# BoloniniD/CSWin-UNet

Hardware: AMD Instinct MI355X
Metric: training images/sec (224x224, cswin_tiny) (higher is better)
Workload: dtype f32; 1 GPU; cswin_tiny_224_lite, synthetic 224x224 9-class, bs=24/GPU, fp32 matmul, fwd + 0.4CE+0.6Dice + bwd + SGD(momentum) step, drop_path 0.2; global_batch=24, img_size=224, parallelism=dp1, hip_graph=True

## Files before the change

### cswin_unet_amd/_lib.py

```python
import ctypes
import os
from ctypes import c_char_p, c_double, c_float, c_int, c_long, c_size_t, c_void_p

import torch

_HERE = os.path.dirname(os.path.abspath(__file__))
LIB_PATH = os.path.join(_HERE, "libcswin_hip.so")

P, I, F, SZ, L, D = c_void_p, c_int, c_float, c_size_t, c_long, c_double

ABI_VERSION = 4

SIGNATURES = {
    "cswin_last_error": (c_char_p, []),
    "cswin_abi_version": (I, []),
    "cswin_device_ok": (I, []),
    "cswin_attn_fwd": (I, [P, P, P, P, P, P, I, I, I, I, P, P, I, F, F, ctypes.c_ulonglong, P, I, P]),
    "cswin_attn_bwd_workspace": (SZ, [I, I, I, I, P, P, I]),
    "cswin_attn_bwd": (I, [P, P, P, P, P, P, P, P, P, P, SZ, I, I, I, I, P, P, I, F, P, F, ctypes.c_ulonglong, P, I, P]),
    "cswin_img2windows": (I, [P, P, I, I, I, I, I, I, P]),
    "cswin_windows2img": (I, [P, P, I, I, I, I, I, I, P]),
    "cswin_layernorm_fwd": (I, [P, P, P, P, P, P, I, I, F, I, P]),
    "cswin_layernorm_bwd_workspace": (SZ, [I, I]),
    "cswin_layernorm_bwd": (I, [P, P, P, P, P, P, P, P, P, P, SZ, I, I, P, P, P]),
    "cswin_linear_fwd": (I, [P, P, I, P, P, P, P, P, P, I, I, I, I, I, I, P]),
    "cswin_linear_bwd_data": (I, [P, P, P, P, I, P, P, I, P, I, I, I, I, I, P]),
    "cswin_linear_bwd_weight_workspace": (SZ, [I, I, I]),
    "cswin_linear_bwd_weight": (I, [P, P, P, I, P, I, P, P, P, SZ, I, I, I, P, I, P]),
    "cswin_linear_bwd_weight_batch": (I, [P, I, P, P, I, P]),
    "cswin_linear_bwd_tail": (I, [P, P, P, I, I, I, P, I, P, P, I, P]),
    "cswin_linear_bwd_weight_batch_masked": (I, [P, I, P, P, I, P, P, P]),
    "cswin_linear_bwd_tail_masked": (I, [P, P, P, I, I, I, P, I, P, P, I, P, P, P]),
    "cswin_rows_sum_multi": (I, [P, I, P]),
    "cswin_conv_tok_fwd": (I, [P, P, P, P, I, I, I, I, I, I, I, I, I, P]),
    "cswin_conv_tok_bwd_data": (I, [P, P, P, I, I, I, I, I, I, I, I, I, P]),
    "cswin_conv_tok_bwd_weight_workspace": (SZ, [I, I, I, I, I, I, I, I]),
    "cswin_conv_tok_bwd_weight": (I, [P, P, P, P, P, SZ, I, I, I, I, I, I, I, I, I, P, I, P]),
    "cswin_conv_weight_permute": (I, [P, P, P, I, I, I, I, P]),
    "cswin_conv_weight_unpermute": (I, [P, P, I, I, I, I, P]),
    "cswin_conv_weight_flipT": (I, [P, P, I, I, I, P]),
# ... 195 lines not shown
```

### cswin_unet_amd/csrc/gemm.hip

```cpp
#include <stdlib.h>

#include <type_traits>
#include "common.h"
#include "gemm_epilogue.h"

int cswin_gemm16(int mode, int epi_mode, const void* A, const void* B, const void* epilogue, int M, int NO, int R, void* stream);
int cswin_wgrad16_batch(const cswin_wgrad_desc* d, int n, const int* splits, const int* rows_per_split, const cswin_reduce_job* pending,
                        int npending, void* stream, long long* stamps);

namespace {

constexpr int BKMAX = 64;

typedef __bf16 bf16x8 __attribute__((ext_vector_type(8)));

#define CSWIN_CHECK_PRECISION(p, who) CSWIN_REQUIRE((p) == 0 || (p) == 1, CSWIN_ERR_UNSUPPORTED, who ": precision %d (0 = fp32, 1 = bf16 operands)", (p))

struct PlainSrc {
    const float* p; long ld; int rows, cols;
    const float* row_scale; int rows_per_sample;
    int bf16;
    static constexpr bool fast_div = false;
    struct Row { const float* base; float s; };
    typedef int Col;
// ... 10 lines not shown
template <class S> __device__ __forceinline__ bool src_is_bf16(const S&) { return false; }
__device__ __forceinline__ bool src_is_bf16(const PlainSrc& s) { return s.bf16 != 0; }
template <class S> __device__ __forceinline__ u32x2 src_load4_bf16(const S&, const float*) { return u32x2{0u, 0u}; }
__device__ __forceinline__ u32x2 src_load4_bf16(const PlainSrc& s, const float* p) {
    return *reinterpret_cast<const u32x2*>(reinterpret_cast<const __bf16*>(s.p) + (p - s.p));
}
template <class S> __device__ __forceinline__ typename S::Row src_mapped_row(const S&, int, float) { return typename S::Row{}; }
__device__ __forceinline__ PlainSrc::Row src_mapped_row(const PlainSrc& s, int row, float f) {
    PlainSrc::Row r;
    r.base = row >= 0 ? s.p + (long)row * s.ld : nullptr;
    r.s = f;
    return r;
}
template <class S> __device__ __forceinline__ const float* src_row_scale(const S&) { return nullptr; }
__device__ __forceinline__ const float* src_row_scale(const PlainSrc& s) { return s.row_scale; }

struct ConcatSrc {
    const float* p0; const float* p1; long ld0, ld1; int rows, cols, c0;
    static constexpr bool fast_div = false;
    struct Row { const float* b0; const float* b1; float s; };
    typedef int Col;
    __device__ Col col(int j) const { return j; }
    __device__ Row row(int i) const {
        Row r;
        r.b0 = (i < rows) ? p0 + (long)i * ld0 : nullptr;
        r.b1 = (i < rows) ? p1 + (long)i * ld1 : nullptr;
        r.s = 1.0f;
        return r;
    }
    __device__ const float* ptr(const Row& r, int j) const {
// ... 140 lines not shown
    constexpr int NW = (BM >= 64 ? 2 : 1) * (BN >= 64 ? 2 : 1);
    constexpr int LDR = BK + 4;
    constexpr int A_ELEMS = A_RC ? BM * LDR : BK * (BM + 4);
    constexpr int B_ELEMS = B_RC ? BN * LDR : BK * (BN + 4);
    return (A_ELEMS + B_ELEMS) > NW * EP_WAVE_FLOATS ? (A_ELEMS + B_ELEMS) : NW * EP_WAVE_FLOATS;
}

struct RowMask { const float* skip; int nsamples, rows_per_sample, splits; unsigned magic; };
constexpr int MASK_MAX_SAMPLES = 256;
struct KeptList { int n; int idx[MASK_MAX_SAMPLES]; float scale[MASK_MAX_SAMPLES]; };

template <int BM, int BN, int BK, int KW, bool A_RC, bool B_RC, int VEC, int EPI, bool SCALE_A, int PREC, class ASrc, class BSrc,
          bool MASKED = false>
__device__ __forceinline__ void gemm_body(float* lds, const ASrc& A, const BSrc& B, const Epilogue& epi, int M, int N, int R,
                                          int r_per_split, int tiles_m, int tiles_n, int bid, int nblk, int stamp_row,
                                          const RowMask* mk = nullptr, KeptList* kept = nullptr) {
    constexpr int WGM = BM >= 64 ? 2 : 1, WGN = BN >= 64 ? 2 : 1, NW = WGM * WGN;
    constexpr int WM = BM / WGM, WN = BN / WGN;
    constexpr int FM = WM / 32, FN = WN / 32;
    constexpr int LDR = BK + 4;
    constexpr int LDA = A_RC ? LDR : BM + 4;
    constexpr int LDB = B_RC ? LDR : BN + 4;
    constexpr int A_ELEMS = A_RC ? BM * LDR : BK * (BM + 4);
    constexpr int B_ELEMS = B_RC ? BN * LDR : BK * (BN + 4);
    constexpr int LDS_FLOATS = gemm_lds_floats<BM, BN, BK, KW, A_RC, B_RC>();
    static_assert(LDS_FLOATS >= A_ELEMS + B_ELEMS && LDS_FLOATS >= NW * EP_WAVE_FLOATS, "gemm_lds_floats out of step with the tile geometry");
    float* As = lds;
    float* Bs = lds + A_ELEMS;
    constexpr int LD16 = BK + 8;
    unsigned short* As16 = reinterpret_cast<unsigned short*>(lds);
    unsigned short* Bs16 = As16 + BM * LD16;
// ... 47 lines not shown
    if (A_RC) {
#pragma unroll
        for (int q = 0; q < QA; ++q) arow[q] = A.row(m0 + a_r + q * A_RPP);
    }
    if (B_RC) {
#pragma unroll
        for (int q = 0; q < QB; ++q) brow[q] = B.row(n0 + b_r + q * B_RPP);
    }

    const typename ASrc::Col acol = A.col(m0 + 4 * a_c);
    const typename BSrc::Col bcol = B.col(n0 + 4 * b_c);

    f32x4 pa[QA], pb[QB];
    u32x2 pa16[QA], pb16[QB];
    float pas[QA];
    auto fetch = [&](int r0, auto a16, auto b16) {
        int mrow[QA];
        float msc[QA];
        if constexpr (MASKED) {
#pragma unroll
            for (int q = 0; q < QA; ++q) {
                const int c = r0 + a_r + q * A_RPP;
                mrow[q] = -1;
                msc[q] = 1.0f;
                if (c < r_end) {
                    const int j = fdiv1(c, mk->magic);
                    mrow[q] = kept->idx[j] * mk->rows_per_sample + (c - j * mk->rows_per_sample);
                    msc[q] = kept->scale[j];
                }
            }
        }
#pragma unroll
        for (int q = 0; q < QA; ++q) {
// ... 75 lines not shown
                    if (SCALE_A) v *= pas[q];
                    const u32x2 u = __builtin_bit_cast(u32x2, __builtin_convertvector(v, bf16x4));
                    h01 = u[0]; h23 = u[1];
                }
                if (A_RC) {
                    *reinterpret_cast<u32x2*>(&As16[(a_r + q * A_RPP) * LD16 + 4 * a_c]) = u32x2{h01, h23};
                } else {
                    unsigned short* col = &As16[4 * a_c * LD16 + a_r + q * A_RPP];
                    col[0] = (unsigned short)(h01 & 0xffffu);
                    col[LD16] = (unsigned short)(h01 >> 16);
                    col[2 * LD16] = (unsigned short)(h23 & 0xffffu);
                    col[3 * LD16] = (unsigned short)(h23 >> 16);
                }
            } else {
                if (SCALE_A) v *= pas[q];
                *reinterpret_cast<f32x4*>(&As[(a_r + q * A_RPP) * LDA + 4 * a_c]) = v;
            }
        }
#pragma unroll
        for (int q = 0; q < QB; ++q) {
            if constexpr (PREC == 1) {
                u32x2 hb;
                if constexpr (decltype(b16)::value) hb = pb16[q];
                else hb = __builtin_bit_cast(u32x2, __builtin_convertvector(pb[q], bf16x4));
                if (B_RC) {
                    *reinterpret_cast<u32x2*>(&Bs16[(b_r + q * B_RPP) * LD16 + 4 * b_c]) = hb;
                } else {
                    static_assert(B_RC || BN == 64, "transposed-read B image is laid out for 64-column tiles");
                    const int row = b_r + q * B_RPP;
                    *reinterpret_cast<u32x2*>(&Bs16[row * BN + 8 * ((b_c >> 1) ^ (((row >> 1) & 1) << 2)) + 4 * (b_c & 1)]) = hb;
// ... 3 lines not shown
            }
        }
    };

    f32x16 acc[FM][FN];
#pragma unroll
    for (int i = 0; i < FM; ++i)
#pragma unroll
        for (int j = 0; j < FN; ++j)
#pragma unroll
            for (int e = 0; e < 16; ++e) acc[i][j][e] = 0.f;

    float csum = 0.f;
    const bool do_colsum = !A_RC && epi.colsum && n0 == 0 && tid < BM;

    if (epi.stamps && tid == 0) { epi.stamps[8L * stamp_row + 0] = __builtin_amdgcn_s_memtime(); epi.stamps[8L * stamp_row + 4] = __builtin_amdgcn_s_getreg(6164); epi.stamps[8L * stamp_row + 5] = __builtin_amdgcn_s_memrealtime(); }
    auto main_loop = [&](auto a16, auto b16) {
        fetch(r_begin, a16, b16);
        stash(a16, b16);
        __syncthreads();
        if (epi.stamps && tid == 0) epi.stamps[8L * stamp_row + 1] = __builtin_amdgcn_s_memtime();
        for (int r0 = r_begin; r0 < r_end; r0 += BK) {
            const bool more = r0 + BK < r_end;
            if (more) fetch(r0 + BK, a16, b16);
            if (do_colsum) {
                if constexpr (PREC == 1) {
#pragma unroll 8
                    for (int r = 0; r < BK; ++r)
                        csum += __builtin_bit_cast(float, (unsigned)As16[tid * LD16 + r] << 16);
                } else {
#pragma unroll 8
                    for (int r = 0; r < BK; ++r) csum += As[r * LDA + tid];
                }
// ... 123 lines not shown
        else
            run_epilogue<EPI, FM, FN>(e, acc, M, N, m0 + wm0, n0 + wn0, lane, lds + wave * EP_WAVE_FLOATS, e.vec_store != 0);
    }
    if (epi.stamps && tid == 0) { epi.stamps[8L * stamp_row + 3] = __builtin_amdgcn_s_memtime(); epi.stamps[8L * stamp_row + 6] = __builtin_amdgcn_s_memrealtime(); }
    if (do_colsum && m0 + tid < M) epi.colsum[(long)split * epi.colsum_stride + m0 + tid] = csum;
}

constexpr int gemm_threads(int BM, int BN, int KW) { return 64 * (BM >= 64 ? 2 : 1) * (BN >= 64 ? 2 : 1) * KW; }

template <int BM, int BN, int BK, int KW, bool A_RC, bool B_RC, int VEC, int EPI, bool SCALE_A, int PREC, class ASrc, class BSrc>
__global__ __launch_bounds__(gemm_threads(BM, BN, KW)) void gemm_kernel(ASrc A, BSrc B, Epilogue epi, int M, int N, int R,
                                                    int r_per_split, int tiles_m, int tiles_n) {
    __shared__ __attribute__((aligned(16))) float lds[gemm_lds_floats<BM, BN, BK, KW, A_RC, B_RC>()];
    gemm_body<BM, BN, BK, KW, A_RC, B_RC, VEC, EPI, SCALE_A, PREC, ASrc, BSrc>(lds, A, B, epi, M, N, R, r_per_split, tiles_m, tiles_n,
                                                                              (int)blockIdx.x, (int)gridDim.x, (int)blockIdx.x);
}

constexpr int WGRAD_BATCH = 4;
template <class ASrc, class BSrc>
struct GemmBatch {
    ASrc A[WGRAD_BATCH];
    BSrc B[WGRAD_BATCH];
    Epilogue e[WGRAD_BATCH];
    int M[WGRAD_BATCH], N[WGRAD_BATCH], R[WGRAD_BATCH], rps[WGRAD_BATCH], tm[WGRAD_BATCH], tn[WGRAD_BATCH];
    int first[WGRAD_BATCH + 1];
    int n;
    RowMask mask[WGRAD_BATCH];
};
typedef GemmBatch<PlainSrc, PlainSrc> WgradBatch;

// ... 75 lines not shown
__global__ __launch_bounds__(256 * KW) void gemm_conv_s2_dgrad_batch_kernel(GemmBatch<ConvTS2SrcT<FAST>, TapRowsSrcT<FAST>> b) {
    int p = 0;
    while (p + 1 < b.n && (int)blockIdx.x >= b.first[p + 1]) ++p;
    __shared__ __attribute__((aligned(16))) float lds[gemm_lds_floats<64, 64, (KW == 1 ? 32 : 64), KW, true, false>()];
    gemm_body<64, 64, (KW == 1 ? 32 : 64), KW, true, false, 4, EPI_PLAIN, false, PREC, ConvTS2SrcT<FAST>, TapRowsSrcT<FAST>>(
        lds, b.A[p], b.B[p], b.e[p], b.M[p], b.N[p], b.R[p], b.rps[p], b.tm[p], b.tn[p], (int)blockIdx.x - b.first[p],
        b.first[p + 1] - b.first[p], (int)blockIdx.x);
}

template <int BM, int BN, int BK, int KW, bool A_RC, bool B_RC, int VEC, int EPI, bool SCALE_A, int PREC, class ASrc, class BSrc>
void launch_cfg(const ASrc& A, const BSrc& B, const Epilogue& epi, int M, int N, int R, int splits, int r_per_split,
                hipStream_t st) {
    int tm = cdiv(M, BM), tn = cdiv(N, BN);
    dim3 grid(tm * tn * splits);
    const int pad_lds = cswin_tuning().gemm_pad_lds;
    hipLaunchKernelGGL((gemm_kernel<BM, BN, BK, KW, A_RC, B_RC, VEC, EPI, SCALE_A, PREC, ASrc, BSrc>), grid, dim3(gemm_threads(BM, BN, KW)), pad_lds, st, A, B, epi,
                       M, N, R, r_per_split, tm, tn);
}

int k_groups(long blocks, int r_len) {
    if (blocks < 320 && r_len >= 512) return 4;
    if (blocks < 640 && r_len >= 256) return 2;
    return 1;
}

int one_split(int R) { return cdiv(R, BKMAX) * BKMAX; }

template <bool A_RC, bool B_RC, int VEC, int EPI, bool SCALE_A, class ASrc, class BSrc>
void launch_gemm(const ASrc& A, const BSrc& B, const Epilogue& epi_in, int M, int N, int R, int splits, int r_per_split,
                 int precision, hipStream_t st) {
    Epilogue epi = epi_in;
    epi.vec_store = epilogue_vec_ok(epi, N);
    auto blocks = [&](int bm, int bn) { return (long)cdiv(M, bm) * cdiv(N, bn) * splits; };
    const int forced_kw = cswin_tuning().gemm_kw;
    const int forced_tile = cswin_tuning().gemm_tile;
    const double pen2 = cswin_tuning().gemm_pen2;
    auto cost = [&](int bm, int bn, double pen) { return (double)((blocks(bm, bn) + 255) / 256) * bm * bn * pen; };
    int tile = 1;
    if (splits == 1 && cost(64, 32, pen2) < cost(64, 64, 1.0)) tile = 2;
    if (forced_tile) tile = forced_tile;
    const int r_len = r_per_split < R ? r_per_split : R;
    const bool wgrad = !A_RC && !B_RC;
    if (precision == 1) {
        if (k_groups(blocks(64, 64), r_len) >= 2 || (wgrad && r_len >= 256))
            launch_cfg<64, 64, 64, 2, A_RC, B_RC, VEC, EPI, SCALE_A, 1>(A, B, epi, M, N, R, splits, r_per_split, st);
        else launch_cfg<64, 64, 64, 1, A_RC, B_RC, VEC, EPI, SCALE_A, 1>(A, B, epi, M, N, R, splits, r_per_split, st);
        return;
    }
    if (tile == 2) {
        if (k_groups(blocks(64, 32), r_len) >= 2)
            return launch_cfg<64, 32, 64, 2, A_RC, B_RC, VEC, EPI, SCALE_A, 0>(A, B, epi, M, N, R, splits, r_per_split, st);
        return launch_cfg<64, 32, 32, 1, A_RC, B_RC, VEC, EPI, SCALE_A, 0>(A, B, epi, M, N, R, splits, r_per_split, st);
    }
    int kw = k_groups(blocks(64, 64), r_len);
    if (wgrad && r_len >= 256 && kw < 2) kw = 2;
    if (forced_kw) kw = forced_kw;
    if (kw == 4) launch_cfg<64, 64, 64, 4, A_RC, B_RC, VEC, EPI, SCALE_A, 0>(A, B, epi, M, N, R, splits, r_per_split, st);
    else if (kw == 2) launch_cfg<64, 64, 64, 2, A_RC, B_RC, VEC, EPI, SCALE_A, 0>(A, B, epi, M, N, R, splits, r_per_split, st);
    else launch_cfg<64, 64, 32, 1, A_RC, B_RC, VEC, EPI, SCALE_A, 0>(A, B, epi, M, N, R, splits, r_per_split, st);
}

template <bool A_RC, bool B_RC, int EPI, bool SCALE_A, class ASrc, class BSrc>
void launch_gemm_vec(bool vec, const ASrc& A, const BSrc& B, const Epilogue& epi, int M, int N, int R, int splits, int r_per_split,
                     int precision, hipStream_t st) {
    if (vec) launch_gemm<A_RC, B_RC, 4, EPI, SCALE_A>(A, B, epi, M, N, R, splits, r_per_split, precision, st);
    else launch_gemm<A_RC, B_RC, 1, EPI, SCALE_A>(A, B, epi, M, N, R, splits, r_per_split, precision, st);
}

long long* g_stamps = nullptr;

Epilogue plain_epilogue(float* C, long ldc) {
    Epilogue e = {};
    e.C = C;
// ... 311 lines not shown
                return CSWIN_OK;
            }
        }
        PlainSrc A = {x, K, M, K, nullptr, 1, io_bf16 & 1};
        bool vec = (K % 4 == 0) && aligned16(x) && aligned16(w);
        CSWIN_REQUIRE(io_bf16 == 0 || (vec && aligned16(y) && (!y_act || aligned16(y_act)) && (!bias || aligned16(bias))), CSWIN_ERR_ALIGN,
                      "linear_fwd: bf16 storage needs 16-B aligned operands");
        if (y_act) launch_gemm_vec<true, true, EPI_ACT, false>(vec, A, B, e, M, N, K, 1, rk, precision, st);
        else if (residual) launch_gemm_vec<true, true, EPI_RES, false>(vec, A, B, e, M, N, K, 1, rk, precision, st);
        else launch_gemm_vec<true, true, EPI_PLAIN, false>(vec, A, B, e, M, N, K, 1, rk, precision, st);
    }
    CSWIN_LAUNCH_CHECK();
    return CSWIN_OK;
}

int cswin_linear_bwd_data(const float* dy, const float* w, float* dx, float* dx2, int k_split, const float* gelu_pre,
                          const float* row_scale, int rows_per_sample, const float* add, int M, int N, int K,
                          int precision, int io_bf16, void* stream) {
    CSWIN_CHECK_PRECISION(precision, "linear_bwd_data");
    CSWIN_REQUIRE(io_bf16 == 0 || (precision == 1 && ((!dx2 && !add) || (io_bf16 & ~4) == 0) && (io_bf16 & ~15) == 0 && K % 4 == 0 && N % 4 == 0), CSWIN_ERR_UNSUPPORTED,
                  "linear_bwd_data: bf16 storage (io_bf16 = %d: 1 = dy, 2 = dx, 4 = w, 8 = gelu_pre) needs precision 1, K and N multiples of 4; split / add outputs take only the weight flag", io_bf16);
    CSWIN_REQUIRE(dy && w && dx && M > 0 && N > 0 && K > 0, CSWIN_ERR_SHAPE, "linear_bwd_data: bad arguments");
    CSWIN_REQUIRE(!dx2 || (k_split > 0 && k_split < K), CSWIN_ERR_SHAPE, "linear_bwd_data: bad concat split");
    CSWIN_REQUIRE(!row_scale || rows_per_sample > 0, CSWIN_ERR_SHAPE, "linear_bwd_data: rows_per_sample must be > 0");
    hipStream_t st = (hipStream_t)stream;
    Epilogue e = plain_epilogue(dx, dx2 ? k_split : K);
    e.C2 = dx2; e.ldc2 = K - k_split; e.col_split = dx2 ? k_split : 0;
    e.gelu_pre = gelu_pre; e.ldpre = K;
    e.row_scale = row_scale; e.rows_per_sample = rows_per_sample;
    e.residual = add; e.ldres = K;
// ... 178 lines not shown
```

### cswin_unet_amd/csrc/gemm_epilogue.h

```cpp
#pragma once
#include "common.h"

namespace {

__device__ __forceinline__ f32x4 widen_bf16x4(u32x2 raw) {
    return f32x4{__builtin_bit_cast(float, raw[0] << 16), __builtin_bit_cast(float, raw[0] & 0xffff0000u),
                 __builtin_bit_cast(float, raw[1] << 16), __builtin_bit_cast(float, raw[1] & 0xffff0000u)};
}
__device__ __forceinline__ void epi_store4(float* base, long idx, f32x4 v, int bf16) {
    if (bf16) *reinterpret_cast<bf16x4*>(reinterpret_cast<__bf16*>(base) + idx) = __builtin_convertvector(v, bf16x4);
    else *reinterpret_cast<f32x4*>(base + idx) = v;
}

enum { EPI_PLAIN = 0, EPI_ACT = 1, EPI_RES = 2, EPI_GELUBWD = 3, EPI_SPLIT2 = 4 };

struct Epilogue {
    float* C; long ldc;
    float* C2; long ldc2; int col_split;
    const float* bias;
    float* Cact; long ldact;
    const float* residual; long ldres;
    const float* row_scale; int rows_per_sample;
    const float* gelu_pre; long ldpre;
    long split_stride;
    float* colsum; int colsum_stride;
    int rm_on, rm_H, rm_W, rm_H2, rm_W2, rm_py, rm_px;
    int vec_store;
    int c_bf16;
    int pre_bf16;
    long long* stamps;
};

constexpr int EP_LD = 36;
constexpr int EP_WAVE_FLOATS = 32 * EP_LD;

template <int EPI, int FM, int FN, bool PRE16 = false, bool FDIV = false>
__device__ __forceinline__ void run_epilogue(const Epilogue& e, f32x16 (&acc)[FM][FN], int M, int N, int mb, int nb,
                                             int lane, float* wbuf, bool vec, unsigned m_hw = 0, unsigned m_w2 = 0) {
    const int li = lane & 31, lh = lane >> 5;
    const int rrow = lane >> 3, rcol = (lane & 7) * 4;
    const bool has_rs = e.row_scale != nullptr;
    auto out_row = [&](int m) -> long {
        if (!e.rm_on) return m;
        const int hw = e.rm_H2 * e.rm_W2;
        int b, jy;
        if constexpr (FDIV) { b = fdiv1(m, m_hw); jy = fdiv1(m - b * hw, m_w2); }
        else { b = m / hw; jy = (m - b * hw) / e.rm_W2; }
        const int rem = m - b * hw;
        return ((long)b * e.rm_H + 2 * jy + e.rm_py) * e.rm_W + 2 * (rem - jy * e.rm_W2) + e.rm_px;
// ... 8 lines not shown
            __builtin_amdgcn_wave_barrier();
            __builtin_amdgcn_fence(__ATOMIC_ACQUIRE, "wavefront");
            const int n = nb + j * 32 + rcol;
            if (vec) {
                f32x4 bias_v = {0.f, 0.f, 0.f, 0.f};
                if (e.bias && n < N) bias_v = *reinterpret_cast<const f32x4*>(e.bias + n);
                f32x4 v[4], aux[4];
                u32x2 aux16[4];
                float rs[4];
#pragma unroll
                for (int p = 0; p < 4; ++p) {
                    const int m = mb + i * 32 + rrow + 8 * p;
                    const bool ok = m < M && n < N;
                    v[p] = *reinterpret_cast<const f32x4*>(&wbuf[(rrow + 8 * p) * EP_LD + rcol]);
                    rs[p] = (has_rs && ok) ? e.row_scale[m / e.rows_per_sample] : 1.0f;
                    if (EPI == EPI_RES || EPI == EPI_GELUBWD) {
                        const float* ap = EPI == EPI_RES ? e.residual : e.gelu_pre;
                        const long ld = EPI == EPI_RES ? e.ldres : e.ldpre;
                        aux[p] = f32x4{0.f, 0.f, 0.f, 0.f};
                        aux16[p] = u32x2{0u, 0u};
                        if (ok) {
                            if constexpr (PRE16) aux16[p] = *reinterpret_cast<const u32x2*>(reinterpret_cast<const __bf16*>(ap) + (long)m * ld + n);
                            else aux[p] = *reinterpret_cast<const f32x4*>(ap + (long)m * ld + n);
                        }
                    }
                }
#pragma unroll
                for (int p = 0; p < 4; ++p) {
                    const int m = mb + i * 32 + rrow + 8 * p;
                    if (m >= M || n >= N) continue;
                    f32x4 o = v[p] + bias_v;
                    if (EPI == EPI_GELUBWD) {
                        const f32x4 pre = PRE16 ? widen_bf16x4(aux16[p]) : aux[p];
#pragma unroll
                        for (int c = 0; c < 4; ++c) o[c] *= gelu_grad_f(pre[c]);
                    }
                    if (has_rs) o *= rs[p];
                    if (EPI == EPI_RES) o += aux[p];
                    if (EPI == EPI_SPLIT2 && n >= e.col_split)
                        *reinterpret_cast<f32x4*>(e.C2 + (long)m * e.ldc2 + (n - e.col_split)) = o;
                    else
// ... 6 lines not shown
                    }
                }
            } else {
#pragma unroll
                for (int p = 0; p < 4; ++p) {
                    const int m = mb + i * 32 + rrow + 8 * p;
                    if (m >= M) continue;
                    const float rsv = has_rs ? e.row_scale[m / e.rows_per_sample] : 1.0f;
#pragma unroll
                    for (int c = 0; c < 4; ++c) {
                        const int nn = n + c;
                        if (nn >= N) continue;
                        float o = wbuf[(rrow + 8 * p) * EP_LD + rcol + c] + (e.bias ? e.bias[nn] : 0.f);
                        if (EPI == EPI_GELUBWD) o *= gelu_grad_f(e.gelu_pre[(long)m * e.ldpre + nn]);
                        o *= rsv;
                        if (EPI == EPI_RES) o += e.residual[(long)m * e.ldres + nn];
                        if (EPI == EPI_SPLIT2 && nn >= e.col_split) e.C2[(long)m * e.ldc2 + (nn - e.col_split)] = o;
                        else e.C[out_row(m) * e.ldc + nn] = o;
                        if (EPI == EPI_ACT) e.Cact[(long)m * e.ldact + nn] = gelu_f(o);
                    }
                }
            }
            __builtin_amdgcn_fence(__ATOMIC_RELEASE, "wavefront");
            __builtin_amdgcn_wave_barrier();
        }
    }
}


inline bool aligned16(const void* p) { return (reinterpret_cast<uintptr_t>(p) & 15) == 0; }

// ... 9 lines not shown
```

### cswin_unet_amd/networks/cswin_unet.py

```python
import math

import numpy as np
import torch
import torch.nn as nn
import torch.utils.checkpoint as checkpoint

from .. import ops
from ..layers import DropPath, TokenRearrange, trunc_normal_


def _square_side(n_tokens):
    side = int(math.isqrt(n_tokens))
    if side * side != n_tokens:
        raise ValueError(f"token count {n_tokens} is not a square map")
    return side


class Mlp(nn.Module):
    def __init__(self, in_features, hidden_features=None, out_features=None, act_layer=nn.GELU, drop=0.):
        super().__init__()
        out_features = out_features or in_features
        hidden_features = hidden_features or in_features
        self.fc1 = nn.Linear(in_features, hidden_features)
        self.act = act_layer()
# ... 290 lines not shown
        w_fused, b_fused = ops.head_compose(head.weight, up.out.weight, up.out.bias, cpad)
        mid, z = ops.linear_pair(x, up.down.weight.flatten(1), up.down.bias, w_fused, None)
        e = ops.conv_tokens(mid, up.encoder.weight, up.encoder.bias, side, side, 1, 1)
        return ops.carafe_reassemble_nchw(e, z, b_fused, side, side, up.up_factor, ncls)

    def _conv_specs(self, pe_weight):
        pe = self.stage1_conv_embed[0]
        specs = [(pe_weight, (pe_weight.shape[1] + 3) // 4 * 4, pe.stride[0], pe.padding[0])]
        specs += [(m.conv.weight, m.conv.weight.shape[1], 2, 1) for m in (self.merge1, self.merge2, self.merge3)]
        specs += [(u.encoder.weight, u.encoder.weight.shape[1], 1, 1)
                  for u in (self.upsample4, self.upsample3, self.upsample2, self.upsample1)]
        return specs

    def forward(self, x):
        pe_weight = self.stage1_conv_embed.conv_weight(x)
        with ops.conv_weight_images(self._conv_specs(pe_weight)):
            return self._forward(x, pe_weight)

    def _forward(self, x, pe_weight):
        x = self.forward_features(x, pe_weight)
        self.xb = x
        bound = [x, self.x1, self.x2, self.x3]
        if getattr(self, "detach_decoder_inputs", False) and torch.is_grad_enabled():
            bound = [t.detach().requires_grad_() for t in bound]
        self.dec_in = bound
        x = self.forward_up_features(bound[0])
        return self.up_x4(x)
```

### cswin_unet_amd/ops.py

```python
import ctypes
import math
import types

import numpy as np
import torch
from torch.autograd import Function
from torch.autograd.function import once_differentiable

from ._lib import AugmentDesc, ConvImageJob, CswinHipError, ReduceJob, WgradDesc, act_bf16, call, dev_f32, lib, precision, ptr, shadow_ptr, stream

__all__ = ["layer_norm", "linear", "linear_pair", "mlp", "stripe_attention", "cswin_block", "conv_tokens", "patch_embed_conv", "carafe_reassemble",
           "carafe_reassemble_nchw", "conv_weight_images", "head_compose", "tokens_to_nchw", "matmul_nn", "ce_dice_loss", "continual_loss", "dropout", "img2windows", "windows2img",
           "seg_metrics", "resize_slices", "argmax_zoom_back", "augment_batch", "class_counts", "gaussian_blur"]


MAX_REDUCE_JOBS = 48
TAIL_RIDER_JOBS = 16


class engine_backward:

    def __init__(self, opt=None):
        self._flat = opt.flat_grad if opt is not None else None
        self._slots = {p.data_ptr(): (o, p.numel()) for p, o in zip(opt.params, opt.offsets)} if opt is not None else {}
        self._queue = []
        self._given = set()

    def __enter__(self):
# ... 134 lines not shown

_twins = {}


def _twin_put(t, t16):
    _twins[t.data_ptr()] = (t, t16)


def _twin_take(t):
    e = _twins.pop(t.data_ptr(), None)
    return e[1] if e is not None and e[0]._cdata == t._cdata else None


def clear_twins():
    _twins.clear()


def _wsrc(w):
    if act_bf16() and w.shape[0] % 4 == 0 and w.shape[1] % 4 == 0:
        sp = shadow_ptr(w)
        if sp is not None:
            return sp, 4
    return ptr(w), 0


def _linear_fwd(x, w, b, N, *, dtype=torch.float32, gelu=False, x2=None, residual=None, row_scale=None):
    pw, w16 = w if isinstance(w, tuple) else (ptr(w), 0)
    K1 = x.shape[-1]
    K = K1 + (x2.shape[-1] if x2 is not None else 0)
    y = torch.empty(x.shape[:-1] + (N,), dtype=dtype, device=x.device)
# ... 292 lines not shown
                w2, bb2, *lepe):
        x = dev_f32(x, "block input")
        B, L, C = x.shape
        if L != reso * reso:
            raise ValueError("flatten img_tokens has wrong size")
        dev = x.device
        nb = len(idx)
        lw = [dev_f32(t).view(t.shape[0], 9) for t in lepe[:nb]]
        lb = [dev_f32(t) for t in lepe[nb:]]
        rs1, rs2 = dev_f32(rs1), dev_f32(rs2)
        s16 = act_bf16() and C % 4 == 0
        t16 = torch.bfloat16 if s16 else torch.float32
        E16 = lambda *shape: torch.empty(*shape, dtype=t16, device=dev)
        sq, sp, s1, s2 = (_wsrc(w) if s16 else w for w in (wqkv, wp, w1, w2))
        attn = (reso, split, tuple(idx), tuple(heads), scale, drop, ATTN_MFMA16 if s16 else ATTN_FP32)
        h1, m1, r1 = _layernorm_fwd(x, g1, b1, eps1, t16)
        qkv = _linear_fwd(h1, sq, bqkv, 3 * C, dtype=t16)
        att, lse = E16(B, L, C), torch.empty(B, sum(heads), L, dtype=torch.float32, device=dev)
        att0 = E16(B, L, C) if any(ctx.needs_input_grad) else None
        _attn_fwd(qkv, lw, lb, att, att0, lse, *attn)
        x1 = _linear_fwd(att, sp, bp, C, residual=x, row_scale=rs1)
        h2, m2, r2 = _layernorm_fwd(x1, g2, b2, eps2, t16)
        pre, act = _linear_fwd(h2, s1, bb1, w1.shape[0], dtype=t16, gelu=True)
        y = _linear_fwd(act, s2, bb2, C, residual=x1, row_scale=rs2)
        ctx.save_for_backward(x, m1, r1, h1, qkv, lse, att, att0, x1, m2, r2, h2, pre, act, rs1, rs2, g1, wqkv, wp, g2, w1, w2, *lw, *lb)
        ctx.attn = attn
        ctx.keys = _param_keys(g1, b1, wqkv, bqkv, wp, bp, g2, b2, w1, bb1, w2, bb2, *lepe)
        return y

    @staticmethod
    @once_differentiable
    def backward(ctx, dy):
        (x, m1, r1, h1, qkv, lse, att, att0, x1, m2, r2, h2, pre, act, rs1, rs2, g1, wqkv, wp, g2, w1, w2, *lwb) = ctx.saved_tensors
        nb = len(lwb) // 2
        lw, lb = lwb[:nb], lwb[nb:]
        dy = dev_f32(dy)
        B, L, C = x.shape
        M, Hd = B * L, w1.shape[0]
        dev, h = x.device, lib()
# ... 692 lines not shown
```

### include/cswin_hip.h

```cpp
#ifndef CSWIN_HIP_H
#define CSWIN_HIP_H

#include <stddef.h>

#ifdef __cplusplus
extern "C" {
#endif

#define CSWIN_ABI_VERSION 4

#define CSWIN_OK 0
#define CSWIN_ERR_SHAPE (-1)
#define CSWIN_ERR_ALIGN (-2)
#define CSWIN_ERR_WORKSPACE (-3)
#define CSWIN_ERR_HIP (-4)
#define CSWIN_ERR_UNSUPPORTED (-5)

typedef struct cswin_reduce_job {
    const float* part;
    float* out;
    float* out2;
    long long n_first, n, stride;
    int rows, reserved;
    int conv_kk, conv_cin;
// ... 14 lines not shown
                   const unsigned long long* drop_epoch, int qkv_bf16, void* stream);

int cswin_img2windows(const float* img, float* out, int B, int C, int H, int W, int H_sp, int W_sp, void* stream);
int cswin_windows2img(const float* win, float* out, int B, int C, int H, int W, int H_sp, int W_sp, void* stream);

int cswin_layernorm_fwd(const float* x, const float* gamma, const float* beta, float* y, float* mean, float* rstd,
                        int M, int C, float eps, int y_bf16, void* stream);
size_t cswin_layernorm_bwd_workspace(int M, int C);
int cswin_layernorm_bwd(const float* dy, const float* x, const float* mean, const float* rstd, const float* gamma,
                        const float* dres, float* dx, float* dgamma, float* dbeta, void* workspace, size_t ws_bytes,
                        int M, int C, cswin_reduce_job* deferred, void* dx_bf16, void* stream);

int cswin_linear_fwd(const float* x, const float* x2, int k_split, const float* w, const float* bias, float* y,
                     float* y_act, const float* residual, const float* row_scale, int rows_per_sample, int M, int N,
                     int K, int precision, int io_bf16, void* stream);
int cswin_linear_bwd_data(const float* dy, const float* w, float* dx, float* dx2, int k_split, const float* gelu_pre,
                          const float* row_scale, int rows_per_sample, const float* add, int M, int N, int K,
                          int precision, int io_bf16, void* stream);
size_t cswin_linear_bwd_weight_workspace(int M, int N, int K);
int cswin_linear_bwd_weight(const float* dy, const float* x, const float* x2, int k_split, const float* row_scale,
                            int rows_per_sample, float* dw, float* dbias, void* workspace, size_t ws_bytes, int M,
                            int N, int K, cswin_reduce_job* deferred, int precision, void* stream);
typedef struct cswin_wgrad_desc {
    const float* dy;
    const float* x;
    const float* row_scale;
    float* dw;
    float* dbias;
    void* workspace;
    size_t ws_bytes;
// ... 141 lines not shown
```

Baseline: 1948 images/sec.

## Fuse LayerNorm into forward Linears via residual-epilogue row statistics

The residual Linear epilogue now also writes per-32-column partial mean and M2 statistics, and a new GEMM source applies LayerNorm on the fly while loading A tiles. It combines those partials into mean and rstd in a prologue and writes the normalised h once. This removes the separate LayerNorm forward kernels and a read of the activations in each CSWin block's forward. In exchange it adds a stats buffer, extra LDS and prologue work in the GEMM, a pointer-keyed stats cache across blocks, and a fallback when the k-split form would be chosen.

```diff
diff --git a/cswin_unet_amd/_lib.py b/cswin_unet_amd/_lib.py
--- a/cswin_unet_amd/_lib.py
+++ b/cswin_unet_amd/_lib.py
@@ -24,6 +24,8 @@
     "cswin_layernorm_bwd_workspace": (SZ, [I, I]),
     "cswin_layernorm_bwd": (I, [P, P, P, P, P, P, P, P, P, P, SZ, I, I, P, P, P]),
     "cswin_linear_fwd": (I, [P, P, I, P, P, P, P, P, P, I, I, I, I, I, I, P]),
+    "cswin_linear_fwd_stats": (I, [P, P, I, P, P, P, P, P, P, I, I, I, I, I, I, P, P]),
+    "cswin_ln_linear_fwd": (I, [P, P, P, P, F, P, P, P, P, P, P, P, I, I, I, I, I, P]),
     "cswin_linear_bwd_data": (I, [P, P, P, P, I, P, P, I, P, I, I, I, I, I, P]),
     "cswin_linear_bwd_weight_workspace": (SZ, [I, I, I]),
     "cswin_linear_bwd_weight": (I, [P, P, P, I, P, I, P, P, P, SZ, I, I, I, P, I, P]),
diff --git a/cswin_unet_amd/csrc/gemm.hip b/cswin_unet_amd/csrc/gemm.hip
--- a/cswin_unet_amd/csrc/gemm.hip
+++ b/cswin_unet_amd/csrc/gemm.hip
@@ -7,6 +7,9 @@
 int cswin_gemm16(int mode, int epi_mode, const void* A, const void* B, const void* epilogue, int M, int NO, int R, void* stream);
 int cswin_wgrad16_batch(const cswin_wgrad_desc* d, int n, const int* splits, const int* rows_per_split, const cswin_reduce_job* pending,
                         int npending, void* stream, long long* stamps);
+
+extern "C" int cswin_layernorm_fwd(const float* x, const float* gamma, const float* beta, float* y, float* mean, float* rstd, int M, int C,
+                                   float eps, int y_bf16, void* stream);
 
 namespace {
 
@@ -48,6 +51,28 @@
 }
 template <class S> __device__ __forceinline__ const float* src_row_scale(const S&) { return nullptr; }
 __device__ __forceinline__ const float* src_row_scale(const PlainSrc& s) { return s.row_scale; }
+
+constexpr int LN_MAX_C = 512, LN_MAX_TILES = LN_MAX_C / 32;
+constexpr int LN_LDS_FLOATS = 2 * LN_MAX_C + 2 * 64;
+__constant__ float LN_INV[LN_MAX_TILES] = {1.0f,     1.0f / 2,  1.0f / 3,  1.0f / 4,  1.0f / 5,  1.0f / 6,  1.0f / 7,  1.0f / 8,
+                                           1.0f / 9, 1.0f / 10, 1.0f / 11, 1.0f / 12, 1.0f / 13, 1.0f / 14, 1.0f / 15, 1.0f / 16};
+struct LnSrc {
+    const float* p; long ld; int rows, cols;
+    const float* stats; int ntiles;
+    const float* gamma; const float* beta; float eps;
+    float* h; float* mean; float* rstd;
+    static constexpr bool fast_div = false;
+    struct Row { const float* base; float s; };
+    typedef int Col;
+    __device__ Col col(int j) const { return j; }
+    __device__ Row row(int i) const {
+        Row r;
+        r.base = (i < rows) ? p + (long)i * ld : nullptr;
+        r.s = 1.0f;
+        return r;
+    }
+    __device__ const float* ptr(const Row& r, int j) const { return (r.base && j < cols) ? r.base + j : nullptr; }
+};
 
 struct ConcatSrc {
     const float* p0; const float* p1; long ld0, ld1; int rows, cols, c0;
@@ -218,7 +243,10 @@
           bool MASKED = false>
 __device__ __forceinline__ void gemm_body(float* lds, const ASrc& A, const BSrc& B, const Epilogue& epi, int M, int N, int R,
                                           int r_per_split, int tiles_m, int tiles_n, int bid, int nblk, int stamp_row,
-                                          const RowMask* mk = nullptr, KeptList* kept = nullptr) {
+                                          const RowMask* mk = nullptr, KeptList* kept = nullptr, float* lnbuf = nullptr) {
+    constexpr bool LN = std::is_same<ASrc, LnSrc>::value;
+    static_assert(!LN || (A_RC && B_RC && VEC == 4 && PREC == 0 && !SCALE_A && !MASKED && BM == 64),
+                  "the normalising source serves the fp32 forward Linears with 16-B loaders");
     constexpr int WGM = BM >= 64 ? 2 : 1, WGN = BN >= 64 ? 2 : 1, NW = WGM * WGN;
     constexpr int WM = BM / WGM, WN = BN / WGN;
     constexpr int FM = WM / 32, FN = WN / 32;
@@ -296,9 +324,16 @@
     f32x4 pa[QA], pb[QB];
     u32x2 pa16[QA], pb16[QB];
     float pas[QA];
+    int ln_r0 = 0, ln_turn = n0 / BN;
+    bool ln_write = false;
     auto fetch = [&](int r0, auto a16, auto b16) {
         int mrow[QA];
         float msc[QA];
+        if constexpr (LN) {
+            ln_r0 = r0;
+            ln_write = ln_turn == 0;
+            ln_turn = ln_write ? tiles_n - 1 : ln_turn - 1;
+        }
         if constexpr (MASKED) {
 #pragma unroll
             for (int q = 0; q < QA; ++q) {
@@ -404,6 +439,16 @@
                 }
             } else {
                 if (SCALE_A) v *= pas[q];
+                if constexpr (LN) {
+                    const int j = ln_r0 + 4 * a_c, m = m0 + a_r + q * A_RPP;
+                    if (j < r_end) {
+                        const f32x4 g = *reinterpret_cast<const f32x4*>(&lnbuf[j]);
+                        const f32x4 b = *reinterpret_cast<const f32x4*>(&lnbuf[LN_MAX_C + j]);
+                        const float mu = lnbuf[2 * LN_MAX_C + 2 * (a_r + q * A_RPP)], rs = lnbuf[2 * LN_MAX_C + 2 * (a_r + q * A_RPP) + 1];
+                        v = (v - mu) * rs * g + b;
+                        if (ln_write && m < M) *reinterpret_cast<f32x4*>(A.h + (long)m * A.cols + j) = v;
+                    }
+                }
                 *reinterpret_cast<f32x4*>(&As[(a_r + q * A_RPP) * LDA + 4 * a_c]) = v;
             }
         }
@@ -437,9 +482,60 @@
     float csum = 0.f;
     const bool do_colsum = !A_RC && epi.colsum && n0 == 0 && tid < BM;
 
+    auto ln_prologue = [&]() {
+        if constexpr (LN) {
+            typedef float f32x2 __attribute__((ext_vector_type(2)));
+            constexpr int PER = (64 * LN_MAX_TILES + NTH - 1) / NTH;
+            static_assert(2 * 64 * LN_MAX_TILES <= LDS_FLOATS, "the operand images hold the panel's pairs");
+            float* lstat = lnbuf + 2 * LN_MAX_C;
+            f32x2* lpair = reinterpret_cast<f32x2*>(lds);
+            const f32x2* sp = reinterpret_cast<const f32x2*>(A.stats) + (long)m0 * A.ntiles;
+            const int npair = min(64, M - m0) * A.ntiles;
+            f32x2 st[PER];
+#pragma unroll
+            for (int i = 0; i < PER; ++i) {
+                st[i] = f32x2{0.f, 0.f};
+                if (tid + i * NTH < npair) st[i] = sp[tid + i * NTH];
+            }
+            for (int c = 4 * tid; c < A.cols; c += 4 * NTH) {
+                *reinterpret_cast<f32x4*>(&lnbuf[c]) = *reinterpret_cast<const f32x4*>(A.gamma + c);
+                *reinterpret_cast<f32x4*>(&lnbuf[LN_MAX_C + c]) = *reinterpret_cast<const f32x4*>(A.beta + c);
+            }
+#pragma unroll
+            for (int i = 0; i < PER; ++i)
+                if (tid + i * NTH < npair) lpair[tid + i * NTH] = st[i];
+            __syncthreads();
+            if (tid < 64) {
+                const int m = m0 + tid;
+                float mu = 0.f, rs = 0.f;
+                if (m < M) {
+                    const f32x2* row = lpair + tid * A.ntiles;
+                    const float frame = row[0][0];
+                    float off = 0.f, m2 = row[0][1];
+#pragma nounroll
+                    for (int k = 1; k < A.ntiles; ++k) {
+                        const f32x2 pk = row[k];
+                        const float inv = LN_INV[k];
+                        const float d = (pk[0] - frame) - off;
+                        off += d * inv;
+                        m2 += pk[1] + d * d * ((float)(32 * k) * inv);
+                    }
+                    mu = frame + off;
+                    rs = rsqrtf(m2 * (1.0f / A.cols) + A.eps);
+                    if (n0 == 0) {
+                        A.mean[m] = mu;
+                        A.rstd[m] = rs;
+                    }
+                }
+                *reinterpret_cast<f32x2*>(&lstat[2 * tid]) = f32x2{mu, rs};
+            }
+            __syncthreads();
+        }
+    };
     if (epi.stamps && tid == 0) { epi.stamps[8L * stamp_row + 0] = __builtin_amdgcn_s_memtime(); epi.stamps[8L * stamp_row + 4] = __builtin_amdgcn_s_getreg(6164); epi.stamps[8L * stamp_row + 5] = __builtin_amdgcn_s_memrealtime(); }
     auto main_loop = [&](auto a16, auto b16) {
         fetch(r_begin, a16, b16);
+        if constexpr (LN) ln_prologue();
         stash(a16, b16);
         __syncthreads();
         if (epi.stamps && tid == 0) epi.stamps[8L * stamp_row + 1] = __builtin_amdgcn_s_memtime();
@@ -593,6 +689,16 @@
     __shared__ __attribute__((aligned(16))) float lds[gemm_lds_floats<BM, BN, BK, KW, A_RC, B_RC>()];
     gemm_body<BM, BN, BK, KW, A_RC, B_RC, VEC, EPI, SCALE_A, PREC, ASrc, BSrc>(lds, A, B, epi, M, N, R, r_per_split, tiles_m, tiles_n,
                                                                               (int)blockIdx.x, (int)gridDim.x, (int)blockIdx.x);
+}
+
+template <int BM, int BN, int BK, int KW, int EPI>
+__global__ __launch_bounds__(gemm_threads(BM, BN, KW)) void gemm_ln_kernel(LnSrc A, PlainSrc B, Epilogue epi, int M, int N, int R,
+                                                                           int r_per_split, int tiles_m, int tiles_n) {
+    __shared__ __attribute__((aligned(16))) float lds[gemm_lds_floats<BM, BN, BK, KW, true, true>()];
+    __shared__ __attribute__((aligned(16))) float lnbuf[LN_LDS_FLOATS];
+    gemm_body<BM, BN, BK, KW, true, true, 4, EPI, false, 0, LnSrc, PlainSrc>(lds, A, B, epi, M, N, R, r_per_split, tiles_m, tiles_n,
+                                                                            (int)blockIdx.x, (int)gridDim.x, (int)blockIdx.x, nullptr,
+                                                                            nullptr, lnbuf);
 }
 
 constexpr int WGRAD_BATCH = 4;
@@ -698,6 +804,10 @@
     int tm = cdiv(M, BM), tn = cdiv(N, BN);
     dim3 grid(tm * tn * splits);
     const int pad_lds = cswin_tuning().gemm_pad_lds;
+    if constexpr (std::is_same<ASrc, LnSrc>::value)
+        hipLaunchKernelGGL((gemm_ln_kernel<BM, BN, BK, KW, EPI>), grid, dim3(gemm_threads(BM, BN, KW)), pad_lds, st, A, B, epi, M, N, R,
+                           r_per_split, tm, tn);
+    else
     hipLaunchKernelGGL((gemm_kernel<BM, BN, BK, KW, A_RC, B_RC, VEC, EPI, SCALE_A, PREC, ASrc, BSrc>), grid, dim3(gemm_threads(BM, BN, KW)), pad_lds, st, A, B, epi,
                        M, N, R, r_per_split, tm, tn);
 }
@@ -712,7 +822,7 @@
 
 template <bool A_RC, bool B_RC, int VEC, int EPI, bool SCALE_A, class ASrc, class BSrc>
 void launch_gemm(const ASrc& A, const BSrc& B, const Epilogue& epi_in, int M, int N, int R, int splits, int r_per_split,
-                 int precision, hipStream_t st) {
+                 int precision, hipStream_t st, bool* no_form = nullptr) {
     Epilogue epi = epi_in;
     epi.vec_store = epilogue_vec_ok(epi, N);
     auto blocks = [&](int bm, int bn) { return (long)cdiv(M, bm) * cdiv(N, bn) * splits; };
@@ -725,6 +835,8 @@
     if (forced_tile) tile = forced_tile;
     const int r_len = r_per_split < R ? r_per_split : R;
     const bool wgrad = !A_RC && !B_RC;
+    constexpr bool FP32_ONLY = EPI == EPI_RES_STATS || std::is_same<ASrc, LnSrc>::value;
+    if constexpr (!FP32_ONLY)
     if (precision == 1) {
         if (k_groups(blocks(64, 64), r_len) >= 2 || (wgrad && r_len >= 256))
             launch_cfg<64, 64, 64, 2, A_RC, B_RC, VEC, EPI, SCALE_A, 1>(A, B, epi, M, N, R, splits, r_per_split, st);
@@ -739,8 +851,15 @@
     int kw = k_groups(blocks(64, 64), r_len);
     if (wgrad && r_len >= 256 && kw < 2) kw = 2;
     if (forced_kw) kw = forced_kw;
+    constexpr bool LN_SRC = std::is_same<ASrc, LnSrc>::value;
+    if (LN_SRC && kw == 2) {
+        if (no_form) *no_form = true;
+        return;
+    }
     if (kw == 4) launch_cfg<64, 64, 64, 4, A_RC, B_RC, VEC, EPI, SCALE_A, 0>(A, B, epi, M, N, R, splits, r_per_split, st);
-    else if (kw == 2) launch_cfg<64, 64, 64, 2, A_RC, B_RC, VEC, EPI, SCALE_A, 0>(A, B, epi, M, N, R, splits, r_per_split, st);
+    else if (kw == 2) {
+        if constexpr (!LN_SRC) launch_cfg<64, 64, 64, 2, A_RC, B_RC, VEC, EPI, SCALE_A, 0>(A, B, epi, M, N, R, splits, r_per_split, st);
+    }
     else launch_cfg<64, 64, 32, 1, A_RC, B_RC, VEC, EPI, SCALE_A, 0>(A, B, epi, M, N, R, splits, r_per_split, st);
 }
 
@@ -1082,6 +1201,54 @@
     return CSWIN_OK;
 }
 
+#define CSWIN_REQUIRE_LN_FUSED(who, C)                                                                                                    \
+    CSWIN_REQUIRE(precision == 0 && io_bf16 == 0, CSWIN_ERR_UNSUPPORTED, who ": fp32 only (precision 0, io_bf16 0)");                     \
+    CSWIN_REQUIRE(x && w && y && M > 0 && N > 0 && K > 0, CSWIN_ERR_SHAPE, who ": bad arguments M=%d N=%d K=%d", M, N, K);                \
+    CSWIN_REQUIRE((C) % 32 == 0 && (C) <= LN_MAX_C, CSWIN_ERR_SHAPE, who ": the normalised width %d must be a multiple of 32 up to %d",   \
+                  (C), LN_MAX_C);                                                                                                         \
+    CSWIN_REQUIRE(K % 4 == 0 && aligned16(x) && aligned16(w) && aligned16(stats) && epilogue_vec_ok(e, N), CSWIN_ERR_ALIGN,               \
+                  who ": needs 16-B aligned operands and K, N multiples of 4")
+
+int cswin_linear_fwd_stats(const float* x, const float* x2, int k_split, const float* w, const float* bias, float* y,
+                           float* y_act, const float* residual, const float* row_scale, int rows_per_sample, int M, int N,
+                           int K, int precision, int io_bf16, float* stats, void* stream) {
+    CSWIN_REQUIRE(!x2 && k_split == 0 && !y_act && residual && stats, CSWIN_ERR_UNSUPPORTED,
+                  "linear_fwd_stats: the residual form of a plain input only (x2, y_act NULL; residual, stats given)");
+    CSWIN_REQUIRE(!row_scale || rows_per_sample > 0, CSWIN_ERR_SHAPE, "linear_fwd_stats: rows_per_sample must be > 0");
+    Epilogue e = plain_epilogue(y, N);
+    e.bias = bias;
+    e.residual = residual; e.ldres = N;
+    e.row_scale = row_scale; e.rows_per_sample = rows_per_sample;
+    CSWIN_REQUIRE_LN_FUSED("linear_fwd_stats", N);
+    e.colsum = stats; e.colsum_stride = N / 32;
+    const PlainSrc A = {x, K, M, K, nullptr, 1, 0}, B = {w, K, N, K, nullptr, 1, 0};
+    launch_gemm<true, true, 4, EPI_RES_STATS, false>(A, B, e, M, N, K, 1, one_split(K), 0, (hipStream_t)stream);
+    CSWIN_LAUNCH_CHECK();
+    return CSWIN_OK;
+}
+
+int cswin_ln_linear_fwd(const float* x, const float* stats, const float* gamma, const float* beta, float eps, float* h, float* mean,
+                        float* rstd, const float* w, const float* bias, float* y, float* y_act, int M, int N, int K, int precision,
+                        int io_bf16, void* stream) {
+    CSWIN_REQUIRE(stats && gamma && beta && h && mean && rstd, CSWIN_ERR_SHAPE, "ln_linear_fwd: bad arguments");
+    Epilogue e = plain_epilogue(y, N);
+    e.bias = bias;
+    e.Cact = y_act; e.ldact = N;
+    CSWIN_REQUIRE_LN_FUSED("ln_linear_fwd", K);
+    CSWIN_REQUIRE(aligned16(gamma) && aligned16(beta) && aligned16(h), CSWIN_ERR_ALIGN, "ln_linear_fwd: needs 16-B aligned gamma, beta and h");
+    const LnSrc A = {x, K, M, K, stats, K / 32, gamma, beta, eps, h, mean, rstd};
+    const PlainSrc B = {w, K, N, K, nullptr, 1, 0};
+    bool no_form = false;
+    if (y_act) launch_gemm<true, true, 4, EPI_ACT, false>(A, B, e, M, N, K, 1, one_split(K), 0, (hipStream_t)stream, &no_form);
+    else launch_gemm<true, true, 4, EPI_PLAIN, false>(A, B, e, M, N, K, 1, one_split(K), 0, (hipStream_t)stream, &no_form);
+    CSWIN_LAUNCH_CHECK();
+    if (no_form) {
+        const int rc = cswin_layernorm_fwd(x, gamma, beta, h, mean, rstd, M, K, eps, 0, stream);
+        return rc ? rc : cswin_linear_fwd(h, nullptr, 0, w, bias, y, y_act, nullptr, nullptr, 1, M, N, K, 0, 0, stream);
+    }
+    return CSWIN_OK;
+}
+
 int cswin_linear_bwd_data(const float* dy, const float* w, float* dx, float* dx2, int k_split, const float* gelu_pre,
                           const float* row_scale, int rows_per_sample, const float* add, int M, int N, int K,
                           int precision, int io_bf16, void* stream) {
diff --git a/cswin_unet_amd/csrc/gemm_epilogue.h b/cswin_unet_amd/csrc/gemm_epilogue.h
--- a/cswin_unet_amd/csrc/gemm_epilogue.h
+++ b/cswin_unet_amd/csrc/gemm_epilogue.h
@@ -1,4 +1,6 @@
 #pragma once
+#include <type_traits>
+
 #include "common.h"
 
 namespace {
@@ -12,7 +14,7 @@
     else *reinterpret_cast<f32x4*>(base + idx) = v;
 }
 
-enum { EPI_PLAIN = 0, EPI_ACT = 1, EPI_RES = 2, EPI_GELUBWD = 3, EPI_SPLIT2 = 4 };
+enum { EPI_PLAIN = 0, EPI_ACT = 1, EPI_RES = 2, EPI_GELUBWD = 3, EPI_SPLIT2 = 4, EPI_RES_STATS = 5 };
 
 struct Epilogue {
     float* C; long ldc;
@@ -33,6 +35,16 @@
 
 constexpr int EP_LD = 36;
 constexpr int EP_WAVE_FLOATS = 32 * EP_LD;
+
+__device__ __forceinline__ float row8_sum(float v) {
+    auto dpp = [](float x, auto ctrl) {
+        return __builtin_bit_cast(float, __builtin_amdgcn_update_dpp(0, __builtin_bit_cast(int, x), decltype(ctrl)::value, 0xf, 0xf, false));
+    };
+    v += dpp(v, std::integral_constant<int, 0xB1>{});
+    v += dpp(v, std::integral_constant<int, 0x4E>{});
+    v += dpp(v, std::integral_constant<int, 0x141>{});
+    return v;
+}
 
 template <int EPI, int FM, int FN, bool PRE16 = false, bool FDIV = false>
 __device__ __forceinline__ void run_epilogue(const Epilogue& e, f32x16 (&acc)[FM][FN], int M, int N, int mb, int nb,
@@ -71,9 +83,9 @@
                     const bool ok = m < M && n < N;
                     v[p] = *reinterpret_cast<const f32x4*>(&wbuf[(rrow + 8 * p) * EP_LD + rcol]);
                     rs[p] = (has_rs && ok) ? e.row_scale[m / e.rows_per_sample] : 1.0f;
-                    if (EPI == EPI_RES || EPI == EPI_GELUBWD) {
-                        const float* ap = EPI == EPI_RES ? e.residual : e.gelu_pre;
-                        const long ld = EPI == EPI_RES ? e.ldres : e.ldpre;
+                    if (EPI == EPI_RES || EPI == EPI_RES_STATS || EPI == EPI_GELUBWD) {
+                        const float* ap = EPI != EPI_GELUBWD ? e.residual : e.gelu_pre;
+                        const long ld = EPI != EPI_GELUBWD ? e.ldres : e.ldpre;
                         aux[p] = f32x4{0.f, 0.f, 0.f, 0.f};
                         aux16[p] = u32x2{0u, 0u};
                         if (ok) {
@@ -82,6 +94,27 @@
                         }
                     }
                 }
+                if constexpr (EPI == EPI_RES_STATS) {
+#pragma unroll
+                    for (int p = 0; p < 4; ++p) {
+                        const int m = mb + i * 32 + rrow + 8 * p;
+                        const bool ok = m < M && n < N;
+                        f32x4 o = v[p] + bias_v;
+                        if (has_rs) o *= rs[p];
+                        o += aux[p];
+                        if (ok) *reinterpret_cast<f32x4*>(e.C + (long)m * e.ldc + n) = o;
+                        const float mu0 = row8_sum((o[0] + o[1]) + (o[2] + o[3])) * (1.0f / 32.0f);
+                        const f32x4 d = o - mu0;
+                        const float s1 = row8_sum((d[0] + d[1]) + (d[2] + d[3]));
+                        const float q = row8_sum((d[0] * d[0] + d[1] * d[1]) + (d[2] * d[2] + d[3] * d[3]));
+                        const float mu = mu0 + s1 * (1.0f / 32.0f);
+                        const float m2 = fmaxf(q - s1 * (s1 * (1.0f / 32.0f)), 0.f);
+                        if (ok && (lane & 7) == 0) {
+                            typedef float f32x2 __attribute__((ext_vector_type(2)));
+                            *reinterpret_cast<f32x2*>(e.colsum + ((long)m * e.colsum_stride + (n >> 5)) * 2) = f32x2{mu, m2};
+                        }
+                    }
+                } else
 #pragma unroll
                 for (int p = 0; p < 4; ++p) {
                     const int m = mb + i * 32 + rrow + 8 * p;
@@ -118,7 +151,7 @@
                         float o = wbuf[(rrow + 8 * p) * EP_LD + rcol + c] + (e.bias ? e.bias[nn] : 0.f);
                         if (EPI == EPI_GELUBWD) o *= gelu_grad_f(e.gelu_pre[(long)m * e.ldpre + nn]);
                         o *= rsv;
-                        if (EPI == EPI_RES) o += e.residual[(long)m * e.ldres + nn];
+                        if (EPI == EPI_RES || EPI == EPI_RES_STATS) o += e.residual[(long)m * e.ldres + nn];
                         if (EPI == EPI_SPLIT2 && nn >= e.col_split) e.C2[(long)m * e.ldc2 + (nn - e.col_split)] = o;
                         else e.C[out_row(m) * e.ldc + nn] = o;
                         if (EPI == EPI_ACT) e.Cact[(long)m * e.ldact + nn] = gelu_f(o);
diff --git a/cswin_unet_amd/networks/cswin_unet.py b/cswin_unet_amd/networks/cswin_unet.py
--- a/cswin_unet_amd/networks/cswin_unet.py
+++ b/cswin_unet_amd/networks/cswin_unet.py
@@ -328,7 +328,7 @@
 
     def forward(self, x):
         pe_weight = self.stage1_conv_embed.conv_weight(x)
-        with ops.conv_weight_images(self._conv_specs(pe_weight)):
+        with ops.conv_weight_images(self._conv_specs(pe_weight)), ops.ln_fusion(True):
             return self._forward(x, pe_weight)
 
     def _forward(self, x, pe_weight):
diff --git a/cswin_unet_amd/ops.py b/cswin_unet_amd/ops.py
--- a/cswin_unet_amd/ops.py
+++ b/cswin_unet_amd/ops.py
@@ -1,3 +1,4 @@
+import contextlib
 import ctypes
 import math
 import types
@@ -11,7 +12,7 @@
 
 __all__ = ["layer_norm", "linear", "linear_pair", "mlp", "stripe_attention", "cswin_block", "conv_tokens", "patch_embed_conv", "carafe_reassemble",
            "carafe_reassemble_nchw", "conv_weight_images", "head_compose", "tokens_to_nchw", "matmul_nn", "ce_dice_loss", "continual_loss", "dropout", "img2windows", "windows2img",
-           "seg_metrics", "resize_slices", "argmax_zoom_back", "augment_batch", "class_counts", "gaussian_blur"]
+           "ln_fusion", "seg_metrics", "resize_slices", "argmax_zoom_back", "augment_batch", "class_counts", "gaussian_blur"]
 
 
 MAX_REDUCE_JOBS = 48
@@ -176,6 +177,55 @@
 
 def clear_twins():
     _twins.clear()
+    _ln_stats.clear()
+
+
+_ln_stats = {}
+_ln_fusion = {"on": False}
+ln_fused_launches = {"stats": 0, "ln_linear": 0}
+LN_FUSED_MAX_C = 512
+
+
+@contextlib.contextmanager
+def ln_fusion(on):
+    prev, _ln_fusion["on"] = _ln_fusion["on"], bool(on)
+    try:
+        yield
+    finally:
+        _ln_fusion["on"] = prev
+
+
+def _ln_stats_put(t, stats):
+    _ln_stats[t.data_ptr()] = (t, t._version, stats)
+
+
+def _ln_stats_take(t):
+    e = _ln_stats.pop(t.data_ptr(), None)
+    return e[2] if e is not None and e[0].shape == t.shape and e[1] == t._version == e[0]._version else None
+
+
+def _linear_fwd_stats(x, w, b, N, *, residual, row_scale):
+    K = x.shape[-1]
+    y = torch.empty(x.shape[:-1] + (N,), dtype=torch.float32, device=x.device)
+    stats = torch.empty(y.numel() // N, N // 32, 2, dtype=torch.float32, device=x.device)
+    call("cswin_linear_fwd_stats", ptr(x), None, 0, ptr(w), ptr(b), ptr(y), None, ptr(residual), ptr(row_scale), _rows_per_sample(x),
+         x.numel() // K, N, K, 0, 0, ptr(stats), stream())
+    ln_fused_launches["stats"] += 1
+    return y, stats
+
+
+def _ln_linear_fwd(x, stats, gamma, beta, eps, w, b, N, *, gelu=False):
+    K = x.shape[-1]
+    M = x.numel() // K
+    h = torch.empty_like(x)
+    mean = torch.empty(M, dtype=torch.float32, device=x.device)
+    rstd = torch.empty_like(mean)
+    y = torch.empty(x.shape[:-1] + (N,), dtype=torch.float32, device=x.device)
+    y_act = torch.empty_like(y) if gelu else None
+    call("cswin_ln_linear_fwd", ptr(x), ptr(stats), ptr(gamma), ptr(beta), eps, ptr(h), ptr(mean), ptr(rstd), ptr(w), ptr(b), ptr(y),
+         ptr(y_act), M, N, K, 0, 0, stream())
+    ln_fused_launches["ln_linear"] += 1
+    return (h, mean, rstd, y, y_act) if gelu else (h, mean, rstd, y)
 
 
 def _wsrc(w):
@@ -498,15 +548,26 @@
         E16 = lambda *shape: torch.empty(*shape, dtype=t16, device=dev)
         sq, sp, s1, s2 = (_wsrc(w) if s16 else w for w in (wqkv, wp, w1, w2))
         attn = (reso, split, tuple(idx), tuple(heads), scale, drop, ATTN_MFMA16 if s16 else ATTN_FP32)
-        h1, m1, r1 = _layernorm_fwd(x, g1, b1, eps1, t16)
-        qkv = _linear_fwd(h1, sq, bqkv, 3 * C, dtype=t16)
+        fused = _ln_fusion["on"] and precision() == 0 and not s16 and C % 32 == 0 and C <= LN_FUSED_MAX_C
+        st1 = _ln_stats_take(x) if fused else None
+        if st1 is not None:
+            h1, m1, r1, qkv = _ln_linear_fwd(x, st1, g1, b1, eps1, wqkv, bqkv, 3 * C)
+        else:
+            h1, m1, r1 = _layernorm_fwd(x, g1, b1, eps1, t16)
+            qkv = _linear_fwd(h1, sq, bqkv, 3 * C, dtype=t16)
         att, lse = E16(B, L, C), torch.empty(B, sum(heads), L, dtype=torch.float32, device=dev)
         att0 = E16(B, L, C) if any(ctx.needs_input_grad) else None
         _attn_fwd(qkv, lw, lb, att, att0, lse, *attn)
-        x1 = _linear_fwd(att, sp, bp, C, residual=x, row_scale=rs1)
-        h2, m2, r2 = _layernorm_fwd(x1, g2, b2, eps2, t16)
-        pre, act = _linear_fwd(h2, s1, bb1, w1.shape[0], dtype=t16, gelu=True)
-        y = _linear_fwd(act, s2, bb2, C, residual=x1, row_scale=rs2)
+        if fused:
+            x1, st2 = _linear_fwd_stats(att, wp, bp, C, residual=x, row_scale=rs1)
+            h2, m2, r2, pre, act = _ln_linear_fwd(x1, st2, g2, b2, eps2, w1, bb1, w1.shape[0], gelu=True)
+            y, sty = _linear_fwd_stats(act, w2, bb2, C, residual=x1, row_scale=rs2)
+            _ln_stats_put(y, sty)
+        else:
+            x1 = _linear_fwd(att, sp, bp, C, residual=x, row_scale=rs1)
+            h2, m2, r2 = _layernorm_fwd(x1, g2, b2, eps2, t16)
+            pre, act = _linear_fwd(h2, s1, bb1, w1.shape[0], dtype=t16, gelu=True)
+            y = _linear_fwd(act, s2, bb2, C, residual=x1, row_scale=rs2)
         ctx.save_for_backward(x, m1, r1, h1, qkv, lse, att, att0, x1, m2, r2, h2, pre, act, rs1, rs2, g1, wqkv, wp, g2, w1, w2, *lw, *lb)
         ctx.attn = attn
         ctx.keys = _param_keys(g1, b1, wqkv, bqkv, wp, bp, g2, b2, w1, bb1, w2, bb2, *lepe)
diff --git a/include/cswin_hip.h b/include/cswin_hip.h
--- a/include/cswin_hip.h
+++ b/include/cswin_hip.h
@@ -52,6 +52,12 @@
 int cswin_linear_fwd(const float* x, const float* x2, int k_split, const float* w, const float* bias, float* y,
                      float* y_act, const float* residual, const float* row_scale, int rows_per_sample, int M, int N,
                      int K, int precision, int io_bf16, void* stream);
+int cswin_linear_fwd_stats(const float* x, const float* x2, int k_split, const float* w, const float* bias, float* y,
+                           float* y_act, const float* residual, const float* row_scale, int rows_per_sample, int M, int N,
+                           int K, int precision, int io_bf16, float* stats, void* stream);
+int cswin_ln_linear_fwd(const float* x, const float* stats, const float* gamma, const float* beta, float eps, float* h, float* mean,
+                        float* rstd, const float* w, const float* bias, float* y, float* y_act, int M, int N, int K, int precision,
+                        int io_bf16, void* stream);
 int cswin_linear_bwd_data(const float* dy, const float* w, float* dx, float* dx2, int k_split, const float* gelu_pre,
                           const float* row_scale, int rows_per_sample, const float* add, int M, int N, int K,
                           int precision, int io_bf16, void* stream);
```

New measurement: 1958 images/sec (median of 6 runs). No clear change (+0.5%).
